# rbesenczi/newMSM

Measured on AMD Instinct MI355X. Metric: label-cost evals/sec, higher is better.
Workload: dtype f64; 1 GPU; pairwise sulc (D=1) unary label-cost table, ico6 data grid / ico4 control grid, 19 labels, 48678 evals = 3187573 point samples per step (BASELINE config 2); kind=univariate, simmeasure=correlation, replicas=1

## Files before the change

### newmsm_amd/csrc/cost.cpp

```cpp
#include <algorithm>
#include <chrono>
#include <cmath>
#include <cstdio>
#include <cstdlib>
#include <cstring>

#include "cost_internal.hpp"
#include "host_parallel.hpp"

using namespace msm;

namespace msm {
int ensure_vertex_major(msm_cost *c) {
    if (c->vm_valid) return MSM_OK;
    msm_ctx *ctx = c->ctx;
    const int Ns = c->source->V, D = c->D, R = c->cfw_rows;
    std::vector<double> vm((size_t)Ns * D);
    for (int d = 0; d < D; ++d)
        for (int v = 0; v < Ns; ++v) vm[(size_t)v * D + d] = c->sfeat[(size_t)d * Ns + v];
    MSM_HIP(c->d_sfeat_vm.ensure(vm.size()));
    {
        const int st = upload_staged(ctx, c->d_sfeat_vm.p, vm.data(), sizeof(double) * vm.size());
        if (st) return st;
    }
// ... 144 lines not shown
    MSM_HIP(c->d_absw.ensure(N));
    st = upload_staged(ctx, c->d_maxw.p, mw.data(), sizeof(double) * (size_t)Ns);
    if (st) return st;
    st = apply_weights_dev(ctx, w, c->d_maxw.p, 1, c->d_absw.p);
    if (st) return st;
    c->absw.resize(N);
    MSM_TRY(stage_d2h(ctx, c->absw.data(), c->d_absw.p, sizeof(double) * (size_t)N));
    MSM_TRY(ctx_sync(ctx));
    return MSM_OK;
}

int ensure_unary_table(msm_cost *c) {
    if (c->table_valid) return MSM_OK;
    int st = need(c, c->have_source, "get_source_data()");
    if (st) return st;
    st = need(c, c->L > 0, "labels");
    if (st) return st;
    st = need(c, c->target->d_feat.p != nullptr && c->target->D == c->D, "target features matching the source features");
    if (st) return st;
    msm_ctx *ctx = c->ctx;
    const int N = c->cpgrid->V;
    MSM_HIP(c->d_U.ensure((size_t)c->L * N));
    if (is_ho(c)) {
        MSM_HIP(hipMemsetAsync(c->d_U.p, 0, sizeof(double) * (size_t)c->L * N, ctx->stream));
        c->table_valid = true;
        return MSM_OK;
    }
    st = ensure_rays(c->target);
    if (st) return st;
    UnaryLaunch u;
    u.tree = dev_tree(c->target);
    u.tfeat = c->target->d_feat.p;
    u.D = c->D;
    u.N = N;
    u.L = c->L;
    u.cp = c->cpgrid->d_xyz.p;
    st = ensure_label_rotations(c);
    if (st) return st;
    u.rnl = c->d_rnl.p;
    u.labels = c->d_labels.p;
    u.src = c->source->d_xyz.p;
    u.Nsrc = c->source->V;
    u.sfeat = c->d_sfeat.p;
    u.cfw = c->cfw.empty() ? nullptr : c->d_cfw.p;
    u.cfw_rows = c->cfw_rows;
    u.pptr = c->d_pptr.p;
    u.pidx = c->d_pidx.p;
    u.order = c->d_order.p;
    u.absw = c->d_absw.p;
    u.pmax = c->pmax;
    u.simmeasure = c->p.simmeasure;
    u.percentile = c->p.percentile;
    u.U = c->d_U.p;
    const size_t nsamp = (size_t)c->L * c->pidx.size();
    MSM_HIP(c->d_tval.ensure(nsamp));
    MSM_HIP(c->d_fix_list.ensure(nsamp));
    MSM_HIP(c->d_fix_pt.ensure(3 * nsamp));
    if (!c->d_fix_count.p) MSM_HIP(c->d_fix_count.zero(unary_fix_counter_words(), ctx->stream));
    if (!c->fix_off_valid) {
        std::vector<uint32_t> off;
        unary_fix_offsets(N, c->L, c->pmax, c->pptr.data(), c->order.data(), off);
        MSM_TRY(c->d_fix_off.upload(off.data(), off.size(), ctx));
        MSM_TRY(ctx_sync(ctx));
        c->fix_off_valid = true;
    }
    MSM_HIP(c->d_queues.ensure(N));
    u.ntri = c->target->T;
    u.tval = c->d_tval.p;
    u.fix_list = c->d_fix_list.p;
    u.fix_pt = c->d_fix_pt.p;
    u.fix_cnt = c->d_fix_count.p;
    u.fix_off = c->d_fix_off.p;
    u.redo_list = c->d_queues.p;
    if (c->timing) {
        u.ev_start = c->ev0[c->ev_next];
        u.ev_stop = c->ev1[c->ev_next];
        c->ev_next = (c->ev_next + 1) % (int)c->ev0.size();
        c->ev_count = std::min(c->ev_count + 1, (int)c->ev0.size());
    }
    switch (c->p.kind) {
        case MSM_COST_UNIVARIATE: st = launch_unary_univariate(ctx, u); break;
        case MSM_COST_MULTIVARIATE:
        case MSM_COST_PATCHWISE: {
            {
                st = ensure_vertex_major(c);
                if (st) return st;
                u.sfeat_vm = c->d_sfeat_vm.p;
                u.cfw_vm = c->cfw.empty() ? nullptr : c->d_cfw_vm.p;
            }
            MSM_HIP(c->d_stri.ensure(nsamp));
            MSM_HIP(c->d_sw3.ensure(3 * nsamp));
            UnaryWeightsScratch w{c->d_stri.p, c->d_sw3.p};
            st = launch_unary_multivariate(ctx, u, w, c->p.kind == MSM_COST_PATCHWISE);
            break;
        }
        default: return fail(MSM_ERR_INVALID, "unknown cost kind %d", c->p.kind);
    }
    if (st) return st;
    c->counters[0] += (int64_t)nsamp;
    c->counters[1] += (int64_t)c->L * N;
    c->table_valid = true;
    return MSM_OK;
}

}

extern "C" {

msm_cost *msm_cost_create(msm_ctx *ctx, const msm_cost_params *params) {
    if (!ctx || !params) {
        fail(MSM_ERR_INVALID, "msm_cost_create: null argument");
        return nullptr;
    }
    if (params->kind < MSM_COST_UNIVARIATE || params->kind > MSM_COST_HO_MULTIVARIATE) {
        fail(MSM_ERR_INVALID, "msm_cost_create: unknown cost kind %d", params->kind);
        return nullptr;
    }
    if (params->simmeasure != 1 && params->simmeasure != 2 && params->simmeasure != 4 && params->simmeasure != 5) {
        fail(MSM_ERR_INVALID, "Unknown similarity metric");
        return nullptr;
    }
    if ((params->simmeasure == 4 || params->simmeasure == 5) && !(params->percentile > 0.0 + kEps && params->percentile < 1.0 - kEps)) {
        fail(MSM_ERR_INVALID, "Percentile must be between 0 and 1.");
        return nullptr;
    }
    msm_cost *c = new msm_cost();
    c->ctx = ctx;
    c->p = *params;
    (void)hipSetDevice(ctx->device);
    if (c->d_counters.zero(4, ctx->stream) != hipSuccess) {
        fail(MSM_ERR_HIP, "msm_cost_create: allocation failed");
        delete c;
        return nullptr;
    }
// ... 221 lines not shown
    if (st) return st;
    if (ngroups) *ngroups = c->ngroups;
    if (ptr) std::copy(c->pptr.begin(), c->pptr.end(), ptr);
    if (idx) {
        if ((int64_t)c->pidx.size() > cap) return fail(MSM_ERR_CAPACITY, "patch index buffer too small");
        std::copy(c->pidx.begin(), c->pidx.end(), idx);
    }
    return MSM_OK;
}

int msm_cost_absolute_weights(msm_cost *c, double *absw) {
    if (!c || !absw) return fail(MSM_ERR_INVALID, "msm_cost_absolute_weights: null argument");
    int st = need(c, c->have_source, "get_source_data()");
    if (st) return st;
    std::copy(c->absw.begin(), c->absw.end(), absw);
    return MSM_OK;
}

int msm_cost_unary_table_async(msm_cost *c) {
    if (!c) return fail(MSM_ERR_INVALID, "null cost");
    MSM_TRY(drop_ctx_pending(c->ctx));
    c->table_valid = false;
    c->rotations_valid = false;
    c->h_U.clear();
    return ensure_unary_table(c);
}

int msm_cost_unary_table_fetch(msm_cost *c, double *U) {
    if (!c || !U) return fail(MSM_ERR_INVALID, "msm_cost_unary_table_fetch: null argument");
    MSM_TRY(drop_ctx_pending(c->ctx));
    int st = need(c, c->table_valid, "msm_cost_unary_table_async()");
    if (st) return st;
    msm_ctx *ctx = c->ctx;
    const size_t n = (size_t)c->L * c->cpgrid->V;
    void *mapped = ctx_mapped(ctx, U, sizeof(double) * n);
    if (mapped && reinterpret_cast<uintptr_t>(mapped) % 16 == 0) {
        st = ctx_flag(ctx);
        if (st) return st;
        st = launch_copy_to_mapped(ctx, c->d_U.p, static_cast<double *>(mapped), n, ctx->d_flag_map);
        if (st) return st;
        MSM_TRY(ctx_sync(ctx));
        volatile int *flags = ctx->h_flag;
        if (flags[0] != 0) {
            flags[0] = 0;
            return check_status(ctx, "computeUnaryCosts");
        }
        return MSM_OK;
    }
    MSM_TRY(c->d_U.download(U, n, ctx));
    return check_status(ctx, "computeUnaryCosts");
}

int msm_cost_unary_table(msm_cost *c, double *U) {
    int st = msm_cost_unary_table_async(c);
    if (st) return st;
    return msm_cost_unary_table_fetch(c, U);
}

int msm_cost_unary_batch(msm_cost *c, const int32_t *nodes, const int32_t *labels, int32_t n, double *out) {
    if (!c || !nodes || !labels || !out || n < 0) return fail(MSM_ERR_INVALID, "msm_cost_unary_batch: bad arguments");
    MSM_TRY(drop_ctx_pending(c->ctx));
    if (!c->table_valid || c->h_U.size() != (size_t)c->L * c->cpgrid->V) {
        int st = ensure_unary_table(c);
        if (st) return st;
        c->h_U.resize((size_t)c->L * c->cpgrid->V);
        st = msm_cost_unary_table_fetch(c, c->h_U.data());
        if (st) return st;
    }
    const int N = c->cpgrid->V;
    for (int i = 0; i < n; ++i) {
        if (nodes[i] < 0 || nodes[i] >= N || labels[i] < 0 || labels[i] >= c->L) return fail(MSM_ERR_INVALID, "unary query %d out of range", i);
        out[i] = c->h_U[(size_t)labels[i] * N + nodes[i]];
    }
    return MSM_OK;
}

int msm_cost_enable_timing(msm_cost *c, int enable) {
    if (!c) return fail(MSM_ERR_INVALID, "null cost");
    if (enable && c->ev0.empty()) {
        c->ev0.resize(64);
        c->ev1.resize(64);
        for (size_t i = 0; i < c->ev0.size(); ++i) {
            MSM_HIP(hipEventCreate(&c->ev0[i]));
            MSM_HIP(hipEventCreate(&c->ev1[i]));
        }
    }
    c->timing = enable != 0;
    c->ev_next = 0;
    c->ev_count = 0;
    return MSM_OK;
}

int msm_cost_kernel_times(msm_cost *c, double *ms, int32_t cap, int32_t *n) {
    if (!c || !ms || !n) return fail(MSM_ERR_INVALID, "msm_cost_kernel_times: null argument");
    MSM_TRY(drop_ctx_pending(c->ctx));
    MSM_TRY(ctx_sync(c->ctx));
    const int total = (int)c->ev0.size(), cnt = std::min(c->ev_count, (int)cap);
    for (int k = 0; k < cnt; ++k) {
        const int slot = ((c->ev_next - cnt + k) % total + total) % total;
        float f = 0.f;
        MSM_HIP(hipEventElapsedTime(&f, c->ev0[slot], c->ev1[slot]));
        ms[k] = f;
    }
    *n = cnt;
    return MSM_OK;
}

int msm_cost_counters(msm_cost *c, int64_t counters[4]) {
    if (!c || !counters) return fail(MSM_ERR_INVALID, "msm_cost_counters: null argument");
// ... 10 lines not shown
```

### newmsm_amd/csrc/cost_internal.hpp

```cpp
#pragma once

#include <vector>

#include "devbuf.hpp"
#include "kernels.hpp"

using msm::DevBuf;

struct msm_cost {
    msm_ctx *ctx = nullptr;
    msm_cost_params p{};
    msm_mesh *target = nullptr, *source = nullptr, *cpgrid = nullptr;
    std::vector<double> orig_xyz;
    std::vector<double> ocp_xyz;
    int D = 0;
    std::vector<double> sfeat;
    DevBuf<double> d_sfeat;
    DevBuf<double> d_sfeat_vm, d_cfw_vm;
    bool vm_valid = false;
    std::vector<double> cfw;
    int cfw_rows = 0;
    DevBuf<double> d_cfw;
    std::vector<double> maxsep;
    double mvdmax = 0;
    DevBuf<double> d_maxsep;
    int L = 0;
    std::vector<double> labels, rot;
    DevBuf<double> d_labels, d_rot;
    DevBuf<double> d_rnl, d_moved;
    std::vector<int32_t> triplets, pairs;
    DevBuf<int32_t> d_triplets, d_pairs;
    DevBuf<double> d_orig, d_ocp;
    DevBuf<int32_t> d_cp_tri, d_cp_tid_ptr, d_cp_tid;
    bool cp_conn_valid = false;
    DevBuf<int32_t> d_labeling;
    DevBuf<double> d_clique_out;
    DevBuf<double> d_ho_vals, d_ho_big;
    DevBuf<unsigned> d_ho_pending, d_ho_count;
    DevBuf<int32_t> d_slot_tri;
    DevBuf<int4> d_blk;
    DevBuf<double> d_slot_w, d_slot_sf, d_slot_cw, d_slot_wda, d_tri_frame, d_tri_stat;
    int64_t move_tails = 0;
    struct PendingMove {
        bool valid = false;
        int kind = 0;
        int label = 0;
        double *E = nullptr;
        uint64_t epoch = 0;
        std::vector<int32_t> labeling;
        msm::CliqueArgs a;
        msm::MoveArgs m;
        msm::MoveLabels lab;
    } pending;
    int64_t prefetch_hits = 0, prefetch_drops = 0;
    DevBuf<unsigned> d_defer_list, d_defer_cnt;
    int move_nblk = 0, move_cap = 0, move_parity = 0;
    bool move_valid = false;
    bool have_source = false;
    int ngroups = 0, pmax = 0;
    std::vector<int32_t> pptr, pidx;
    DevBuf<int32_t> d_pptr, d_pidx;
    std::vector<int32_t> order;
    DevBuf<int32_t> d_order;
    DevBuf<uint32_t> d_fix_off;
    bool fix_off_valid = false;
    std::vector<double> absw;
    DevBuf<int32_t> d_pidx_asc;
    DevBuf<uint32_t> d_code;
    DevBuf<double4> d_chunkb;
    bool pidx_asc_on_device = false;
    int patch_cap_hint = 0;
    DevBuf<double> d_absw, d_maxw;
    DevBuf<double> d_U;
    bool table_valid = false;
    bool rotations_valid = false;
    std::vector<double> h_U;
    DevBuf<unsigned long long> d_counters;
    int64_t counters[4] = {0, 0, 0, 0};
    DevBuf<uint32_t> d_slots;
    DevBuf<double> d_tval;
    DevBuf<int> d_stri;
    DevBuf<double> d_sw3;
    DevBuf<unsigned long long> d_fix_list;
    DevBuf<double> d_fix_pt;
    DevBuf<unsigned int> d_fix_count;
    msm_mesh *asphere = nullptr;
    int aVs = 0, aTs = 0;
    DevBuf<double> d_atarget, d_asrc, d_aw_val;
    DevBuf<int32_t> d_asrc_tri, d_aw_ptr, d_aw_cp, d_af_ptr, d_af_idx;
    bool have_anat = false;
    bool timing = false;
    std::vector<hipEvent_t> ev0, ev1;
    int ev_next = 0, ev_count = 0;
    DevBuf<int> d_queues;
    DevBuf<int> d_counts;
};


namespace msm {
int query_host(msm_mesh *target, const double *q, int N, int *tri_id, int *vid, double *w, int mode, const char *what, const double *q_on_device = nullptr);
const Adjacency &mesh_adjacency(msm_mesh *m);
int ensure_label_rotations(msm_cost *c);
int drop_pending_move(msm_cost *c);
int ensure_vertex_major(msm_cost *c);
inline bool cost_is_ho(const msm_cost *c) { return c->p.kind == MSM_COST_HO_UNIVARIATE || c->p.kind == MSM_COST_HO_MULTIVARIATE; }
}
```

### newmsm_amd/csrc/internal.hpp

```cpp
#pragma once

#include <hip/hip_runtime.h>

#include <cstdarg>
#include <cstdint>
#include <cstdio>
#include <functional>
#include <memory>
#include <mutex>
#include <string>
#include <vector>

#include "../../include/msmhip.h"
#include "devbuf.hpp"
#include "geom.hpp"

namespace msm {

void set_error(const char *fmt, ...);
int fail(int code, const char *fmt, ...);
void pool_trim();
size_t pool_idle_bytes();

#define MSM_HIP(call)                                                                                 \
// ... 30 lines not shown
    bool simple = false;
    int G = 0;
    std::vector<int4> cell;
    std::vector<float4> edge;
    std::vector<int4> more;
    std::vector<int4> excl;
    double r2lo = 0, r2hi = 0;
};

struct FlatOctree {
    std::vector<int4> node;
    std::vector<double4> nodebox;
    int nmask_blocks = 0;
    std::vector<int32_t> parent;
    std::vector<int32_t> leaf_tri;
    std::vector<int32_t> grid;
    int grid_depth = 0;
    RayTable rays;
    int64_t stats[5] = {0, 0, 0, 0, 0};
    int dev_nnodes = 0, dev_entries = 0;
    int nnodes() const { return node.empty() ? dev_nnodes : (int)node.size(); }
    int nentries() const { return node.empty() ? dev_entries : (int)leaf_tri.size(); }
};
void build_octree(const double *xyz , const int32_t *tri , int V, int T, FlatOctree &out);
void build_ray_table(const double *xyz, const int32_t *tri, int V, int T, FlatOctree &tree);

struct DevTree {
    const int4 *node;
    const int32_t *parent;
    const int32_t *leaf_tri;
    const float4 *cone;
    const TriRec *rec;
    const int32_t *grid;
    int grid_depth;
    int simple;
    const unsigned long long *mask;
    int nnodes;
    int ray_G;
    const int4 *ray_cell;
    const float4 *ray_tri;
    const int4 *ray_more, *ray_excl;
    double ray_r2lo, ray_r2hi;
};

}

namespace msm {
struct Stager;
}

struct msm_ctx {
    int device = 0;
    int num_cus = 256;
    hipStream_t stream = nullptr;
    bool own_stream = false;
    int *d_status = nullptr;
    int *h_status = nullptr;
    msm::DevBuf<char> q_buf[5];
    msm::Stager *stager = nullptr;
    hipEvent_t wait_ev = nullptr;
    struct msm_cost *pending_cost = nullptr;
    uint64_t epoch = 0;
    void *io_pin = nullptr;
    void *io_dev = nullptr;
    size_t io_cap = 0;
    int *h_flag = nullptr;
    int *d_flag_map = nullptr;
    std::shared_ptr<void> resample_scratch;
    hipEvent_t q_ev0 = nullptr, q_ev1 = nullptr;
    bool q_timing = false, q_timed = false;
    msm::DevBuf<double> oct_box;
    msm::DevBuf<int> oct_ints, oct_counters;
    int *oct_hcounters = nullptr;
    struct HostBlock {
        char *host;
        char *dev;
        size_t bytes;
        bool registered = false;
    };
    std::vector<HostBlock> host_blocks;
};

namespace msm {
struct RayJob;
}

struct msm_mesh {
    msm_ctx *ctx = nullptr;
    int V = 0, T = 0, D = 0;
    std::vector<double> xyz;
    std::vector<int32_t> tri;
    std::vector<double> feat;
    bool tree_valid = false;
    bool gpu_tree_always = false;
    bool host_xyz_stale = false;
    std::shared_ptr<void> oct_job;
    msm::FlatOctree tree;
    bool masks_valid = false;
    bool rays_valid = false;
    bool rayrec_valid = false;
    msm::Adjacency adj;
    bool adj_valid = false;
    msm::DevBuf<double> d_xyz;
    msm::DevBuf<int32_t> d_tri;
    msm::DevBuf<float4> d_tcone;
    msm::DevBuf<double> d_feat;
// ... 84 lines not shown
```

### newmsm_amd/csrc/kernels.hpp

```cpp
#pragma once

#include "internal.hpp"

namespace msm {

int launch_build_masks(msm_ctx *ctx, const DevTree &T, const double4 *d_nodebox, unsigned long long *d_mask);
int launch_build_recs(msm_ctx *ctx, const double *d_xyz, int V, const int32_t *d_tri, int T, TriRec *d_rec, float4 *d_tcone, const int32_t *d_leaf_tri,
                      int nentries, float4 *d_cone);
int launch_build_recs_forest(msm_ctx *ctx, const double *d_xyz, size_t comp_stride, size_t tree_stride, const int32_t *d_tri, int T, int B, TriRec *d_rec, float4 *d_tcone,
                             size_t s_rec, const int32_t *d_leaf_tri, float4 *d_cone, size_t s_leaf, const int *d_entries, size_t entries_stride);
int launch_build_raytri(msm_ctx *ctx, const TriRec *d_rec, const float4 *d_edge, int T, const double *d_feat1, int D, float4 *d_out);
struct AdaptiveDevArgs {
    int nOld, nNew;
    const int *fvid, *rvid;
    const double *fw, *rw;
    const double *oldA, *newA;
    int *roff, *rfill, *rkey;
    double *rwt;
    int *coff, *cfill, *ckey;
    double *cval, *correction;
    int *scan_tmp;
    int *long_flag;
    int *tkey;
    double *tval;
// ... 9 lines not shown
int launch_vertex_areas(msm_ctx *ctx, const double *d_xyz, int V, const int32_t *d_tri, int T, const int32_t *d_tid_ptr, const int32_t *d_tid, double *d_ta,
                        double *d_area);
int launch_adaptive_surgery(msm_ctx *ctx, const AdaptiveDevArgs &a);
int launch_apply_rows(msm_ctx *ctx, int nNew, int nOld, int D, const int *row_ptr, const int *col, const double *val, const double *d_data, double *d_out);
int launch_copy_to_mapped(msm_ctx *ctx, const double *d_src, double *mapped_dst, size_t n, int *flags_mapped);
int launch_query(msm_ctx *ctx, const DevTree &T, const double *d_q, int N, int *d_tri, int *d_vid, double *d_w, int mode);
int launch_query_rays(msm_ctx *ctx, const DevTree &T, const double *d_q, int N, int *d_tri, int *d_vid, double *d_w, int mode, int *d_open);
int launch_closest_vertex(msm_ctx *ctx, const DevTree &T, const double *d_q, int N, int *d_out);
int launch_warp(msm_ctx *ctx, const DevTree &T, const double *d_q, int N, const double *d_to, int V, bool to_sphere, double *d_out);
int query_lanes(long long N);
inline size_t smooth_bounds_offset(int N) { return ((size_t)3 * N + 3) / 4 * 4; }
inline size_t smooth_scratch_doubles(int N) { return smooth_bounds_offset(N) + 4 * (((size_t)N + 63) / 64) + 4; }
int launch_smooth(msm_ctx *ctx, const double *d_xyz, int N, double *d_unit, const int *d_cv, const double *d_data, int Vorig, int D, double sigma,
                  double cosang, const double *d_excl, double *d_out, double *d_excl_out);
int launch_fold_detect(msm_ctx *ctx, const double *d_xyz, int V, const int32_t *d_tri, int T, const int32_t *d_tid_ptr, const int32_t *d_tid, int32_t *d_fold);
int launch_sort_patches(msm_ctx *ctx, const double *d_xyz, int n, const int32_t *d_pptr, int ngroups, const int32_t *d_pidx, uint32_t *d_code,
                        int32_t *d_sorted);
struct RangeGrid {
    const int *start = nullptr, *ids = nullptr, *bad = nullptr;
    int G = 0;
    double origin = 0.0, inv_h = 0.0;
};
int launch_range_grid_build(msm_ctx *ctx, const double *d_src, int Nsrc, int G, double origin, double inv_h, int *d_start, int *d_cursor, int *d_ids, int *d_bad, int *d_tmp);
int launch_range(msm_ctx *ctx, const double *d_cp, int Ncp, const double *d_src, int Nsrc, const double *d_maxsep, double range, int cap,
                 uint32_t *d_slots, int *d_counts, double4 *d_chunk_bounds, int *d_nflag, int cluster = 1, const RangeGrid *grid = nullptr);
int launch_patch_compact(msm_ctx *ctx, const uint32_t *d_slots, int cap, const int32_t *d_pptr, int M, int32_t *d_pidx, size_t pidx_cap = (size_t)-1);
int launch_scan_exclusive(msm_ctx *ctx, int *d_data, int n, int *d_tmp);

int launch_label_rotations(msm_ctx *ctx, const double *d_cp, int N, const double *d_rot, const double *d_labels, int L, double *d_rnl,
                           double *d_moved);

struct UnaryLaunch {
    DevTree tree;
    const double *tfeat;
    int D;
    int N, L;
    const double *cp;
    const double *rnl;
    const double *labels;
    const double *src;
    int Nsrc;
    const double *sfeat;
    const double *cfw;
    int cfw_rows;
    const double *sfeat_vm = nullptr;
    const double *cfw_vm = nullptr;
    const int *pptr, *pidx;
    const int *order;
    const double *absw;
    int pmax;
    int simmeasure;
    double percentile;
    double *U;
    int ntri;
    double *tval;
    unsigned long long *fix_list;
    double *fix_pt;
    unsigned int *fix_cnt;
    const unsigned int *fix_off;
    int *redo_list;
    hipEvent_t ev_start = nullptr, ev_stop = nullptr;
};
int unary_nsplit(int L, int pmax);
int unary_fix_segments();
size_t unary_fix_counter_words();
void unary_fix_offsets(int N, int L, int pmax, const int32_t *pptr, const int32_t *order, std::vector<uint32_t> &off);
int launch_unary_univariate(msm_ctx *ctx, const UnaryLaunch &u);
struct UnaryWeightsScratch {
    int *stri;
    double *sw3;
};
int launch_unary_multivariate(msm_ctx *ctx, const UnaryLaunch &u, const UnaryWeightsScratch &w, bool patchwise);

struct CliqueArgs {
    int kind, simmeasure;
    int N, L, T, P;
    const int *triplets;
    const int *pairs;
    const double *cp;
    const double *ocp;
    const double *orig;
    int Norig;
    const double *moved;
    const double *rnl;
    const int *cp_tri;
    int Tc;
    const int *cp_tid_ptr, *cp_tid;
    double lambda, mu, kappa, k_exp, rexp, mvdmax, percentile;
    DevTree tree;
    const double *tfeat;
    int D;
    const double *src;
    int Nsrc;
    const double *sfeat;
    const double *cfw;
    int cfw_rows;
    const double *sfeat_vm, *cfw_vm;
    const int *bin_ptr, *bin_idx;
    int bin_cap;
    double *ho_big;
    double *ho_vals;
    unsigned *ho_pending;
    unsigned *ho_count;
    const double *absw;
    int rmode;
    DevTree atree;
    const double *atarget;
    int Va;
    const double *asrc;
    int Vs;
    const int *asrc_tri;
    int Ts;
    const int *aw_ptr, *aw_cp;
    const double *aw_val;
    const int *af_ptr, *af_idx;
    int *status;
};
constexpr int kPairSmallPatch = 80;
constexpr int kHoBinMax = 16384;
constexpr int kHoBigBlocks = 512;
// ... 102 lines not shown
```

### newmsm_amd/csrc/unary_kernels.hip

```cpp
#include <algorithm>
#include <cstdlib>

#include "kernels.hpp"
#include "search_device.hpp"
#include "similarity_device.hpp"

#ifndef MSM_VARIANT
#define MSM_VARIANT 0
#endif

namespace msm {

namespace {

constexpr int kFixSegs = 64;
constexpr int kCntStride = 32;
constexpr int kChunk = 768;
constexpr int kQueueCap = 3072;
constexpr int kDeferred = 1 << 20;
constexpr unsigned kInvalidPair = 0xffffffffu;
constexpr int kTriBits = 22;

__device__ __forceinline__ void raise_status(int *status, int code) { atomicMin(status, code); }

__device__ __forceinline__ double wave_sum(double v) {
#pragma unroll
    for (int off = 32; off > 0; off >>= 1) v += __shfl_xor(v, off, 64);
    return v;
}

struct SamplesArgs {
    DevTree tree;
    const double *tfeat;
    int tD;
    int N, L;
    const double *rnl;
    const double *src;
    int Nsrc;
    const int *pptr, *pidx;
    const int *order;
    int pmax;
    int nsplit;
    double *tval;
    int *stri;
    double *sw3;
    unsigned long long *fix_list;
    double *fix_pt;
    unsigned int *fix_cnt;
    const unsigned int *fix_off;
    const double *sfeat;
    const double *cfw;
    const double *absw;
    int simmeasure;
    double percentile;
    double *U;
    int *redo_list;
    unsigned int *redo_count;
    int *status;
// ... 422 lines not shown
            else emit_sample(a, g, p, t);
        }
    }
}

struct ReduceArgs {
    int N, L, Nsrc;
    const double *sfeat;
    const double *cfw;
    int cfw_rows;
    const int *pptr, *pidx;
    const double *absw;
    const double *tval;
    int pmax;
    int simmeasure;
    double percentile;
    double *U;
    const int *redo_list;
    const unsigned int *redo_count;
};

__global__ __launch_bounds__(256) void k_unary_reduce_univariate(ReduceArgs a) {
    extern __shared__ __align__(16) double lds[];
    double *sA = lds, *sW = sA + a.pmax;
    const int tid = threadIdx.x, lane = tid & 63, wave = tid >> 6;
    const unsigned n = a.redo_count ? *a.redo_count : (unsigned)a.N;
    for (unsigned k = blockIdx.x; k < n; k += gridDim.x) {
        const int node = a.redo_list ? a.redo_list[k] : (int)k;
        const int beg = a.pptr[node], P = a.pptr[node + 1] - beg;
        __syncthreads();
        for (int i = tid; i < P; i += 256) {
            const int s = a.pidx[beg + i];
            sA[i] = a.sfeat[s];
            sW[i] = (a.cfw && a.cfw_rows >= 1) ? a.cfw[s] : 1.0;
        }
        __syncthreads();
        const double absw = a.absw[node];
        for (int l = wave; l < a.L; l += 4) {
            const double cost = patch_similarity(sA, sW, a.tval + (size_t)a.L * beg + (size_t)l * P, P, lane, a.simmeasure, a.percentile);
            if (lane == 0) a.U[(size_t)l * a.N + node] = absw * cost;
        }
    }
}

constexpr int kRedLanes = 8;
constexpr int kRedKeep = 12;

__device__ __forceinline__ double group_sum(double v) {
#pragma unroll
    for (int off = kRedLanes / 2; off > 0; off >>= 1) v += __shfl_xor(v, off, kRedLanes);
    return v;
}

__global__ __launch_bounds__(256) void k_unary_reduce_flat(ReduceArgs a, unsigned int *clear, int clear_words) {
    extern __shared__ __align__(16) double lds[];
    double *sA = lds, *sW = sA + a.pmax;
    __shared__ double s_stat[3];
    const int tid = threadIdx.x, sub = tid & (kRedLanes - 1), grp = tid / kRedLanes;
    if (blockIdx.x == 0 && clear)
        for (int k = tid; k < clear_words; k += 256) clear[k] = 0u;
    const int node = a.redo_list ? a.redo_list[blockIdx.x] : (int)blockIdx.x;
    const int beg = a.pptr[node], P = a.pptr[node + 1] - beg;
    const bool has_w = a.cfw && a.cfw_rows >= 1;
    const bool in_regs = true;
    double breg[kRedKeep];
#pragma unroll
    for (int k = 0; k < kRedKeep; ++k) breg[k] = 0.0;
    if (grp < a.L) {
        const double *B = a.tval + (size_t)a.L * beg + (size_t)grp * P;
#pragma unroll
        for (int k = 0; k < kRedKeep; ++k) breg[k] = (sub + kRedLanes * k < P) ? B[sub + kRedLanes * k] : 0.0;
    }
    for (int i = tid; i < P; i += 256) {
        const int s = a.pidx[beg + i];
        sA[i] = a.sfeat[s];
        sW[i] = has_w ? a.cfw[s] : 1.0;
    }
    __syncthreads();
    if (a.simmeasure == 2) {
        if (tid < 64) {
            double sw = 0, ma = 0;
            for (int i = tid; i < P; i += 64) {
                sw += sW[i];
                ma += sW[i] * sA[i];
            }
            sw = wave_sum(sw);
            ma = wave_sum(ma);
            if (sw > 0.0) ma /= sw;
            double va = 0;
            for (int i = tid; i < P; i += 64) {
                const double da = sA[i] - ma;
                va += sW[i] * da * da;
            }
            va = wave_sum(va);
            if (tid == 0) s_stat[0] = sw, s_stat[1] = ma, s_stat[2] = va;
        }
        __syncthreads();
    }
    const double absw = a.absw[node];
    for (int l = grp; l < a.L; l += 256 / kRedLanes) {
        const double *B = a.tval + (size_t)a.L * beg + (size_t)l * P;
        if (!(in_regs && l == grp)) {
#pragma unroll
            for (int k = 0; k < kRedKeep; ++k) breg[k] = (sub + kRedLanes * k < P) ? B[sub + kRedLanes * k] : 0.0;
        }
        double cost;
        if (a.simmeasure == 2) {
            const double sw = s_stat[0], ma = s_stat[1];
            double mb = 0;
#pragma unroll
            for (int k = 0; k < kRedKeep; ++k) {
                const int i = sub + kRedLanes * k;
                if (i < P) mb += sW[i] * breg[k];
            }
            for (int i = sub + kRedLanes * kRedKeep; i < P; i += kRedLanes) mb += sW[i] * B[i];
            mb = group_sum(mb);
            if (sw > 0.0) mb /= sw;
            double pr = 0, vb = 0;
#pragma unroll
            for (int k = 0; k < kRedKeep; ++k) {
                const int i = sub + kRedLanes * k;
                if (i < P) {
                    const double da = sA[i] - ma, db = breg[k] - mb;
                    pr += sW[i] * da * db;
                    vb += sW[i] * db * db;
                }
            }
            for (int i = sub + kRedLanes * kRedKeep; i < P; i += kRedLanes) {
                const double da = sA[i] - ma, db = B[i] - mb;
                pr += sW[i] * da * db;
                vb += sW[i] * db * db;
            }
            pr = group_sum(pr);
            vb = group_sum(vb);
            double va = s_stat[2];
            if (sw > 0.0) {
                pr /= sw;
                va /= sw;
                vb /= sw;
            }
            const double r = (va == 0.0 || vb == 0.0) ? 0.0 : pr / (sqrt(va) * sqrt(vb));
            cost = 1 - (1 + r) * 0.5;
        } else {
            double pr = 0;
#pragma unroll
            for (int k = 0; k < kRedKeep; ++k) {
                const int i = sub + kRedLanes * k;
                if (i < P) {
                    const double df = sA[i] - breg[k];
                    pr += sW[i] * df * df;
                }
            }
            for (int i = sub + kRedLanes * kRedKeep; i < P; i += kRedLanes) {
                const double df = sA[i] - B[i];
                pr += sW[i] * df * df;
            }
            pr = group_sum(pr);
            cost = sqrt(pr) / P;
        }
        if (sub == 0) a.U[(size_t)l * a.N + node] = absw * cost;
    }
}

struct ReduceMvArgs {
    int N, L, Nsrc, D;
    const double *tfeat;
    const TriRec *rec;
    const double *sfeat;
    const double *cfw;
    int cfw_rows;
    const int *pptr, *pidx;
    const double *absw;
    const int *stri;
    const double *sw3;
    int simmeasure;
    double percentile;
    int patchwise;
    int pmax;
    double *U;
};

__global__ __launch_bounds__(256) void k_unary_reduce_features(ReduceMvArgs a) {
    const int node = blockIdx.x;
    const int beg = a.pptr[node], P = a.pptr[node + 1] - beg;
    const int tid = threadIdx.x, lane = tid & 63, wave = tid >> 6;
    const double absw = a.absw[node];
    const double nan = __longlong_as_double(0x7ff8000000000000ll);
    const int nwaves = blockDim.x >> 6;
    for (int l = wave; l < a.L; l += nwaves) {
        const size_t g0 = (size_t)a.L * beg + (size_t)l * P;
        double cost;
        if (!a.patchwise) {
            double acc = 0.0;
            bool bad = false;
            for (int i = lane; i < P; i += 64) {
                const int t = a.stri[g0 + i];
                if (t < 0) {
                    bad = true;
                    continue;
                }
                const TriRec &r = a.rec[t];
                const double *f0 = a.tfeat + (size_t)r.id[0] * a.D, *f1 = a.tfeat + (size_t)r.id[1] * a.D, *f2 = a.tfeat + (size_t)r.id[2] * a.D;
                acc += feature_vector_similarity(a.simmeasure, a.percentile, a.sfeat, a.cfw, a.cfw_rows, a.Nsrc, a.pidx[beg + i], a.D, f0, f1, f2,
                                                 a.sw3[3 * (g0 + i)], a.sw3[3 * (g0 + i) + 1], a.sw3[3 * (g0 + i) + 2]);
            }
            acc = wave_sum(acc);
            cost = P > 0 ? acc / P : acc;
            if (__ballot(bad)) cost = nan;
        } else {
            double total = 0.0;
            bool bad = false;
            for (int d = 0; d < a.D; ++d) {
                const double *A = a.sfeat + (size_t)d * a.Nsrc;
// ... 275 lines not shown

static bool uses_ray_table(const DevTree &t) { return t.simple && t.ray_G > 0 && t.ray_cell && t.ray_tri; }

static int launch_samples(msm_ctx *ctx, const UnaryLaunch &u, const UnaryWeightsScratch *w, SamplesArgs &a, bool fused_reduction = false) {
    if (u.tree.nnodes <= 0 || !u.tree.mask) return fail(MSM_ERR_STATE, "target search structure missing");
    a.tree = u.tree;
    a.tfeat = u.tfeat;
    a.tD = u.D > 0 ? u.D : 1;
    a.N = u.N;
    a.L = u.L;
    a.rnl = u.rnl;
    a.src = u.src;
    a.Nsrc = u.Nsrc;
    a.pptr = u.pptr;
    a.pidx = u.pidx;
    a.order = u.order;
    a.pmax = u.pmax;
    a.tval = w ? nullptr : u.tval;
    a.stri = w ? w->stri : nullptr;
    a.sw3 = w ? w->sw3 : nullptr;
    a.fix_list = u.fix_list;
    a.fix_pt = u.fix_pt;
    a.fix_cnt = u.fix_cnt;
    a.fix_off = u.fix_off;
    a.sfeat = u.sfeat;
    a.cfw = (u.cfw && u.cfw_rows >= 1) ? u.cfw : nullptr;
    a.absw = u.absw;
    a.simmeasure = u.simmeasure;
    a.percentile = u.percentile;
    a.U = (w || !fused_reduction) ? nullptr : u.U;
    a.redo_list = u.redo_list;
    a.redo_count = u.fix_cnt;
    a.status = ctx->d_status;
    if (u.ntri >= (1 << kTriBits)) return fail(MSM_ERR_CAPACITY, "target mesh has %d triangles; the sample queue packs ids in %d bits", u.ntri, kTriBits);
    a.nsplit = unary_nsplit(u.L, u.pmax);
    const size_t lds = samples_lds(u.pmax, u.L, a.nsplit);
    if (!uses_ray_table(u.tree) && lds > 64 * 1024) {
        if (lds > 160 * 1024) return fail(MSM_ERR_CAPACITY, "a patch of %d points does not fit in LDS", u.pmax);
        MSM_HIP(hipFuncSetAttribute(reinterpret_cast<const void *>(k_unary_samples), hipFuncAttributeMaxDynamicSharedMemorySize, (int)lds));
    }
    const int blocks = a.nsplit * 8 * ((u.N + 7) / 8);
    if (u.ev_start) MSM_HIP(hipEventRecord(u.ev_start, ctx->stream));
    if (uses_ray_table(u.tree)) {
        a.U = nullptr;
        const int lper = (u.L + a.nsplit - 1) / a.nsplit;
        const size_t rays_lds = sizeof(double) * (3 * (size_t)u.pmax + 9 * (size_t)u.L) + sizeof(int) * ((size_t)lper * u.pmax + 4) + 16;
        if (rays_lds > 64 * 1024) MSM_HIP(hipFuncSetAttribute(reinterpret_cast<const void *>(k_unary_rays), hipFuncAttributeMaxDynamicSharedMemorySize, (int)rays_lds));
        hipLaunchKernelGGL(k_unary_rays, dim3(blocks), dim3(256), rays_lds, ctx->stream, a);
    } else {
        hipLaunchKernelGGL(k_unary_samples, dim3(blocks), dim3(256), lds, ctx->stream, a);
    }
    MSM_HIP(hipGetLastError());
    if (u.ev_stop) MSM_HIP(hipEventRecord(u.ev_stop, ctx->stream));
    hipLaunchKernelGGL(k_unary_fixup, dim3(4096), dim3(256), 0, ctx->stream, a);
    MSM_HIP(hipGetLastError());
    return MSM_OK;
}

int launch_unary_univariate(msm_ctx *ctx, const UnaryLaunch &u) {
    SamplesArgs a;
    const bool dice = u.simmeasure == 4 || u.simmeasure == 5;
    int st = launch_samples(ctx, u, nullptr, a, dice);
    if (st) return st;
    ReduceArgs r;
    r.N = u.N;
    r.L = u.L;
    r.Nsrc = u.Nsrc;
    r.sfeat = u.sfeat;
    r.cfw = u.cfw;
    r.cfw_rows = u.cfw_rows;
    r.pptr = u.pptr;
    r.pidx = u.pidx;
    r.absw = u.absw;
    r.tval = u.tval;
    r.pmax = u.pmax;
    r.simmeasure = u.simmeasure;
    r.percentile = u.percentile;
    r.U = u.U;
    r.redo_list = u.redo_list;
    r.redo_count = u.fix_cnt;
    if (uses_ray_table(u.tree) && dice) {
        r.redo_list = nullptr;
        r.redo_count = nullptr;
        hipLaunchKernelGGL(k_unary_reduce_univariate, dim3(std::min(u.N, 2048)), dim3(256), sizeof(double) * 2 * (size_t)u.pmax, ctx->stream, r);
        MSM_HIP(hipMemsetAsync(u.fix_cnt, 0, unary_fix_counter_words() * sizeof(unsigned), ctx->stream));
    } else if (!dice) {
        r.redo_list = u.order;
        hipLaunchKernelGGL(k_unary_reduce_flat, dim3(u.N), dim3(256), sizeof(double) * 2 * (size_t)u.pmax, ctx->stream, r, u.fix_cnt,
                           (int)unary_fix_counter_words());
    } else {
        hipLaunchKernelGGL(k_unary_reduce_univariate, dim3(64), dim3(256), sizeof(double) * 2 * (size_t)u.pmax, ctx->stream, r);
        MSM_HIP(hipMemsetAsync(u.fix_cnt, 0, unary_fix_counter_words() * sizeof(unsigned), ctx->stream));
    }
    MSM_HIP(hipGetLastError());
    return MSM_OK;
}

int launch_unary_multivariate(msm_ctx *ctx, const UnaryLaunch &u, const UnaryWeightsScratch &w, bool patchwise) {
    SamplesArgs a;
    int st = launch_samples(ctx, u, &w, a);
    if (st) return st;
    ReduceMvArgs r;
    r.N = u.N;
    r.L = u.L;
    r.Nsrc = u.Nsrc;
    r.D = u.D;
    r.tfeat = u.tfeat;
    r.rec = u.tree.rec;
    r.sfeat = u.sfeat;
    r.cfw = u.cfw;
    r.cfw_rows = u.cfw_rows;
    r.pptr = u.pptr;
    r.pidx = u.pidx;
    r.absw = u.absw;
    r.stri = w.stri;
    r.sw3 = w.sw3;
    r.simmeasure = u.simmeasure;
    r.patchwise = patchwise ? 1 : 0;
    r.pmax = u.pmax;
    r.percentile = u.percentile;
    r.U = u.U;
    const bool dice = u.simmeasure == 4 || u.simmeasure == 5;
    if (!dice && u.D >= 12 && u.D <= kMvLanes * kMvKeep && u.sfeat_vm) {
        ReduceMv8Args m;
        m.N = u.N, m.L = u.L, m.Nsrc = u.Nsrc, m.D = u.D;
        m.tfeat = u.tfeat;
        m.rec = u.tree.rec;
        m.sfeat_vm = u.sfeat_vm;
        m.cfw_vm = u.cfw_vm;
        m.cfw_rows = u.cfw_rows;
        m.pptr = u.pptr, m.pidx = u.pidx, m.order = u.order;
        m.absw = u.absw;
        m.stri = w.stri, m.sw3 = w.sw3;
        m.simmeasure = u.simmeasure;
        m.U = u.U;
        if (!patchwise) hipLaunchKernelGGL(k_unary_reduce_mv8, dim3(u.N), dim3(256), 0, ctx->stream, m);
        else if (u.D <= 32) hipLaunchKernelGGL(k_unary_reduce_pw8<4>, dim3(u.N), dim3(256), 0, ctx->stream, m);
        else hipLaunchKernelGGL(k_unary_reduce_pw8<8>, dim3(u.N), dim3(256), 0, ctx->stream, m);
// ... 18 lines not shown
```

Baseline: 367.2 million evals/s.

## Tile univariate reduce across nodes and write table directly to mapped host memory

Adds a k_unary_finish kernel that reduces several control nodes per block, staging per-label costs in LDS and prefetching the next row's samples into registers. It also clears the fixup counters and reports status, replacing the separate reduce launch and memset. When the caller's output buffer is host-mapped, the kernel writes results straight into it, skipping the separate copy-to-mapped launch or download. The fixup kernel grid is now sized to resident occupancy instead of a fixed 4096 blocks. The cost is that the whole table is written over system memory from the kernel, and the new kernel uses more LDS per block.

New measurement: 355.6 million evals/s. -3.2%, worse.

```diff
diff --git a/newmsm_amd/csrc/cost.cpp b/newmsm_amd/csrc/cost.cpp
--- a/newmsm_amd/csrc/cost.cpp
+++ b/newmsm_amd/csrc/cost.cpp
@@ -220,6 +220,9 @@
     u.simmeasure = c->p.simmeasure;
     u.percentile = c->p.percentile;
     u.U = c->d_U.p;
+    u.U_mapped = c->deliver_to;
+    u.flag_mapped = ctx->d_flag_map;
+    c->delivered = false;
     const size_t nsamp = (size_t)c->L * c->pidx.size();
     MSM_HIP(c->d_tval.ensure(nsamp));
     MSM_HIP(c->d_fix_list.ensure(nsamp));
@@ -247,7 +250,7 @@
         c->ev_count = std::min(c->ev_count + 1, (int)c->ev0.size());
     }
     switch (c->p.kind) {
-        case MSM_COST_UNIVARIATE: st = launch_unary_univariate(ctx, u); break;
+        case MSM_COST_UNIVARIATE: st = launch_unary_univariate(ctx, u, &c->delivered); break;
         case MSM_COST_MULTIVARIATE:
         case MSM_COST_PATCHWISE: {
             {
@@ -575,9 +578,29 @@
 }
 
 int msm_cost_unary_table(msm_cost *c, double *U) {
+    if (!c || !U) return fail(MSM_ERR_INVALID, "msm_cost_unary_table: null argument");
+    msm_ctx *ctx = c->ctx;
+    c->deliver_to = nullptr;
+    c->delivered = false;
+    if (c->cpgrid && c->L > 0) {
+        void *mapped = ctx_mapped(ctx, U, sizeof(double) * (size_t)c->L * c->cpgrid->V);
+        if (mapped && reinterpret_cast<uintptr_t>(mapped) % 16 == 0) {
+            int st = ctx_flag(ctx);
+            if (st) return st;
+            c->deliver_to = static_cast<double *>(mapped);
+        }
+    }
     int st = msm_cost_unary_table_async(c);
-    if (st) return st;
-    return msm_cost_unary_table_fetch(c, U);
+    c->deliver_to = nullptr;
+    if (st) return st;
+    if (!c->delivered) return msm_cost_unary_table_fetch(c, U);
+    MSM_TRY(ctx_sync(ctx));
+    volatile int *flags = ctx->h_flag;
+    if (flags[0] != 0) {
+        flags[0] = 0;
+        return check_status(ctx, "computeUnaryCosts");
+    }
+    return MSM_OK;
 }
 
 int msm_cost_unary_batch(msm_cost *c, const int32_t *nodes, const int32_t *labels, int32_t n, double *out) {
diff --git a/newmsm_amd/csrc/cost_internal.hpp b/newmsm_amd/csrc/cost_internal.hpp
--- a/newmsm_amd/csrc/cost_internal.hpp
+++ b/newmsm_amd/csrc/cost_internal.hpp
@@ -74,6 +74,8 @@
     DevBuf<double> d_U;
     bool table_valid = false;
     bool rotations_valid = false;
+    double *deliver_to = nullptr;
+    bool delivered = false;
     std::vector<double> h_U;
     DevBuf<unsigned long long> d_counters;
     int64_t counters[4] = {0, 0, 0, 0};
diff --git a/newmsm_amd/csrc/internal.hpp b/newmsm_amd/csrc/internal.hpp
--- a/newmsm_amd/csrc/internal.hpp
+++ b/newmsm_amd/csrc/internal.hpp
@@ -106,6 +106,7 @@
 struct msm_ctx {
     int device = 0;
     int num_cus = 256;
+    int unary_fixup_blocks = 0;
     hipStream_t stream = nullptr;
     bool own_stream = false;
     int *d_status = nullptr;
diff --git a/newmsm_amd/csrc/kernels.hpp b/newmsm_amd/csrc/kernels.hpp
--- a/newmsm_amd/csrc/kernels.hpp
+++ b/newmsm_amd/csrc/kernels.hpp
@@ -85,6 +85,8 @@
     int simmeasure;
     double percentile;
     double *U;
+    double *U_mapped = nullptr;
+    int *flag_mapped = nullptr;
     int ntri;
     double *tval;
     unsigned long long *fix_list;
@@ -98,7 +100,7 @@
 int unary_fix_segments();
 size_t unary_fix_counter_words();
 void unary_fix_offsets(int N, int L, int pmax, const int32_t *pptr, const int32_t *order, std::vector<uint32_t> &off);
-int launch_unary_univariate(msm_ctx *ctx, const UnaryLaunch &u);
+int launch_unary_univariate(msm_ctx *ctx, const UnaryLaunch &u, bool *delivered = nullptr);
 struct UnaryWeightsScratch {
     int *stri;
     double *sw3;
diff --git a/newmsm_amd/csrc/unary_kernels.hip b/newmsm_amd/csrc/unary_kernels.hip
--- a/newmsm_amd/csrc/unary_kernels.hip
+++ b/newmsm_amd/csrc/unary_kernels.hip
@@ -4,6 +4,7 @@
 #include "kernels.hpp"
 #include "search_device.hpp"
 #include "similarity_device.hpp"
+#include "unary_shape.hpp"
 
 #ifndef MSM_VARIANT
 #define MSM_VARIANT 0
@@ -532,6 +533,88 @@
     return v;
 }
 
+__device__ __forceinline__ void flat_patch_stats(const double *sA, const double *sW, int P, int lane, double *stat) {
+    double sw = 0, ma = 0;
+    for (int i = lane; i < P; i += 64) {
+        sw += sW[i];
+        ma += sW[i] * sA[i];
+    }
+    sw = wave_sum(sw);
+    ma = wave_sum(ma);
+    if (sw > 0.0) ma /= sw;
+    double va = 0;
+    for (int i = lane; i < P; i += 64) {
+        const double da = sA[i] - ma;
+        va += sW[i] * da * da;
+    }
+    va = wave_sum(va);
+    if (lane == 0) stat[0] = sw, stat[1] = ma, stat[2] = va;
+}
+
+__device__ __forceinline__ void flat_row_load(double (&breg)[kRedKeep], const double *B, int P, int sub) {
+#pragma unroll
+    for (int k = 0; k < kRedKeep; ++k) breg[k] = (sub + kRedLanes * k < P) ? B[sub + kRedLanes * k] : 0.0;
+}
+
+__device__ __forceinline__ double flat_row_cost(int simmeasure, const double *sA, const double *sW, const double (&breg)[kRedKeep], const double *B, int P,
+                                                int sub, const double *stat) {
+    double cost;
+    if (simmeasure == 2) {
+        const double sw = stat[0], ma = stat[1];
+        double mb = 0;
+#pragma unroll
+        for (int k = 0; k < kRedKeep; ++k) {
+            const int i = sub + kRedLanes * k;
+            if (i < P) mb += sW[i] * breg[k];
+        }
+        for (int i = sub + kRedLanes * kRedKeep; i < P; i += kRedLanes) mb += sW[i] * B[i];
+        mb = group_sum(mb);
+        if (sw > 0.0) mb /= sw;
+        double pr = 0, vb = 0;
+#pragma unroll
+        for (int k = 0; k < kRedKeep; ++k) {
+            const int i = sub + kRedLanes * k;
+            if (i < P) {
+                const double da = sA[i] - ma, db = breg[k] - mb;
+                pr += sW[i] * da * db;
+                vb += sW[i] * db * db;
+            }
+        }
+        for (int i = sub + kRedLanes * kRedKeep; i < P; i += kRedLanes) {
+            const double da = sA[i] - ma, db = B[i] - mb;
+            pr += sW[i] * da * db;
+            vb += sW[i] * db * db;
+        }
+        pr = group_sum(pr);
+        vb = group_sum(vb);
+        double va = stat[2];
+        if (sw > 0.0) {
+            pr /= sw;
+            va /= sw;
+            vb /= sw;
+        }
+        const double r = (va == 0.0 || vb == 0.0) ? 0.0 : pr / (sqrt(va) * sqrt(vb));
+        cost = 1 - (1 + r) * 0.5;
+    } else {
+        double pr = 0;
+#pragma unroll
+        for (int k = 0; k < kRedKeep; ++k) {
+            const int i = sub + kRedLanes * k;
+            if (i < P) {
+                const double df = sA[i] - breg[k];
+                pr += sW[i] * df * df;
+            }
+        }
+        for (int i = sub + kRedLanes * kRedKeep; i < P; i += kRedLanes) {
+            const double df = sA[i] - B[i];
+            pr += sW[i] * df * df;
+        }
+        pr = group_sum(pr);
+        cost = sqrt(pr) / P;
+    }
+    return cost;
+}
+
 __global__ __launch_bounds__(256) void k_unary_reduce_flat(ReduceArgs a, unsigned int *clear, int clear_words) {
     extern __shared__ __align__(16) double lds[];
     double *sA = lds, *sW = sA + a.pmax;
@@ -547,9 +630,7 @@
 #pragma unroll
     for (int k = 0; k < kRedKeep; ++k) breg[k] = 0.0;
     if (grp < a.L) {
-        const double *B = a.tval + (size_t)a.L * beg + (size_t)grp * P;
-#pragma unroll
-        for (int k = 0; k < kRedKeep; ++k) breg[k] = (sub + kRedLanes * k < P) ? B[sub + kRedLanes * k] : 0.0;
+        flat_row_load(breg, a.tval + (size_t)a.L * beg + (size_t)grp * P, P, sub);
     }
     for (int i = tid; i < P; i += 256) {
         const int s = a.pidx[beg + i];
@@ -558,87 +639,108 @@
     }
     __syncthreads();
     if (a.simmeasure == 2) {
-        if (tid < 64) {
-            double sw = 0, ma = 0;
-            for (int i = tid; i < P; i += 64) {
-                sw += sW[i];
-                ma += sW[i] * sA[i];
-            }
-            sw = wave_sum(sw);
-            ma = wave_sum(ma);
-            if (sw > 0.0) ma /= sw;
-            double va = 0;
-            for (int i = tid; i < P; i += 64) {
-                const double da = sA[i] - ma;
-                va += sW[i] * da * da;
-            }
-            va = wave_sum(va);
-            if (tid == 0) s_stat[0] = sw, s_stat[1] = ma, s_stat[2] = va;
-        }
+        if (tid < 64) flat_patch_stats(sA, sW, P, tid, s_stat);
         __syncthreads();
     }
     const double absw = a.absw[node];
     for (int l = grp; l < a.L; l += 256 / kRedLanes) {
         const double *B = a.tval + (size_t)a.L * beg + (size_t)l * P;
-        if (!(in_regs && l == grp)) {
-#pragma unroll
-            for (int k = 0; k < kRedKeep; ++k) breg[k] = (sub + kRedLanes * k < P) ? B[sub + kRedLanes * k] : 0.0;
-        }
-        double cost;
-        if (a.simmeasure == 2) {
-            const double sw = s_stat[0], ma = s_stat[1];
-            double mb = 0;
-#pragma unroll
-            for (int k = 0; k < kRedKeep; ++k) {
-                const int i = sub + kRedLanes * k;
-                if (i < P) mb += sW[i] * breg[k];
-            }
-            for (int i = sub + kRedLanes * kRedKeep; i < P; i += kRedLanes) mb += sW[i] * B[i];
-            mb = group_sum(mb);
-            if (sw > 0.0) mb /= sw;
-            double pr = 0, vb = 0;
-#pragma unroll
-            for (int k = 0; k < kRedKeep; ++k) {
-                const int i = sub + kRedLanes * k;
-                if (i < P) {
-                    const double da = sA[i] - ma, db = breg[k] - mb;
-                    pr += sW[i] * da * db;
-                    vb += sW[i] * db * db;
-                }
-            }
-            for (int i = sub + kRedLanes * kRedKeep; i < P; i += kRedLanes) {
-                const double da = sA[i] - ma, db = B[i] - mb;
-                pr += sW[i] * da * db;
-                vb += sW[i] * db * db;
-            }
-            pr = group_sum(pr);
-            vb = group_sum(vb);
-            double va = s_stat[2];
-            if (sw > 0.0) {
-                pr /= sw;
-                va /= sw;
-                vb /= sw;
-            }
-            const double r = (va == 0.0 || vb == 0.0) ? 0.0 : pr / (sqrt(va) * sqrt(vb));
-            cost = 1 - (1 + r) * 0.5;
+        if (!(in_regs && l == grp)) flat_row_load(breg, B, P, sub);
+        const double cost = flat_row_cost(a.simmeasure, sA, sW, breg, B, P, sub, s_stat);
+        if (sub == 0) a.U[(size_t)l * a.N + node] = absw * cost;
+    }
+}
+
+struct FinishOut {
+    double *mapped;
+    const int *status;
+    int *flags;
+    unsigned int *clear;
+    int clear_words;
+};
+
+#ifndef MSM_FINISH_TILE
+#define MSM_FINISH_TILE 8
+#endif
+constexpr int kFinishTile = MSM_FINISH_TILE;
+
+template <int TILE>
+__global__ __launch_bounds__(64 * TILE, 4) void k_unary_finish(ReduceArgs a, FinishOut o) {
+    extern __shared__ __align__(16) double lds[];
+    constexpr int kGroups = 8 * TILE, kThreads = 64 * TILE;
+    double *sU = lds, *sStat = sU + (size_t)a.L * TILE, *sA = sStat + 4 * TILE, *sW = sA + (size_t)TILE * a.pmax;
+    const int tid = threadIdx.x, sub = tid & (kRedLanes - 1), grp = tid / kRedLanes, lane = tid & 63, wave = tid >> 6;
+    if (blockIdx.x == 0) {
+        for (int k = tid; k < o.clear_words; k += kThreads) o.clear[k] = 0u;
+        if (o.mapped && tid == 0) {
+            const int st = *o.status;
+            if (st != 0) __hip_atomic_store(o.flags, st, __ATOMIC_RELAXED, __HIP_MEMORY_SCOPE_SYSTEM);
+        }
+    }
+    const int node0 = blockIdx.x * TILE, nt = min(TILE, a.N - node0), rows = nt * a.L;
+    const int beg0 = a.pptr[node0];
+    const bool has_w = a.cfw && a.cfw_rows >= 1;
+    int w = 0, l = 0, off = 0, P = 0;
+    const double *B = a.tval;
+    auto locate = [&](int r) {
+        w = r / a.L;
+        l = r - w * a.L;
+        const int beg = a.pptr[node0 + w];
+        P = a.pptr[node0 + w + 1] - beg;
+        off = beg - beg0;
+        B = a.tval + (size_t)a.L * beg + (size_t)l * P;
+    };
+    double breg[kRedKeep], bnext[kRedKeep];
+#pragma unroll
+    for (int k = 0; k < kRedKeep; ++k) breg[k] = bnext[k] = 0.0;
+    if (grp < rows) {
+        locate(grp);
+        flat_row_load(breg, B, P, sub);
+    }
+    const int total = a.pptr[node0 + nt] - beg0;
+    for (int i = tid; i < total; i += kThreads) {
+        const int s = a.pidx[beg0 + i];
+        sA[i] = a.sfeat[s];
+        sW[i] = has_w ? a.cfw[s] : 1.0;
+    }
+    __syncthreads();
+    if (a.simmeasure == 2) {
+        for (int k = wave; k < nt; k += TILE) {
+            const int beg = a.pptr[node0 + k];
+            flat_patch_stats(sA + (beg - beg0), sW + (beg - beg0), a.pptr[node0 + k + 1] - beg, lane, sStat + 4 * k);
+        }
+        __syncthreads();
+    }
+    for (int r = grp; r < rows; r += kGroups) {
+        const int w_now = w, l_now = l, off_now = off, P_now = P;
+        const double *B_now = B;
+        if (r + kGroups < rows) {
+            locate(r + kGroups);
+            flat_row_load(bnext, B, P, sub);
+        }
+        const double cost = flat_row_cost(a.simmeasure, sA + off_now, sW + off_now, breg, B_now, P_now, sub, sStat + 4 * w_now);
+        if (sub == 0) sU[l_now * TILE + w_now] = a.absw[node0 + w_now] * cost;
+#pragma unroll
+        for (int k = 0; k < kRedKeep; ++k) breg[k] = bnext[k];
+    }
+    __syncthreads();
+    for (int t = tid; t < a.L * (TILE / 2); t += kThreads) {
+        const int ls = t / (TILE / 2), h = t - ls * (TILE / 2);
+        const size_t at = (size_t)ls * a.N + node0 + 2 * h;
+        const double2 v = *reinterpret_cast<const double2 *>(sU + ls * TILE + 2 * h);
+        if (unary_finish_wide_store(ls, a.N, node0, nt, TILE)) {
+            *reinterpret_cast<double2 *>(a.U + at) = v;
+            if (o.mapped) *reinterpret_cast<double2 *>(o.mapped + at) = v;
         } else {
-            double pr = 0;
-#pragma unroll
-            for (int k = 0; k < kRedKeep; ++k) {
-                const int i = sub + kRedLanes * k;
-                if (i < P) {
-                    const double df = sA[i] - breg[k];
-                    pr += sW[i] * df * df;
-                }
-            }
-            for (int i = sub + kRedLanes * kRedKeep; i < P; i += kRedLanes) {
-                const double df = sA[i] - B[i];
-                pr += sW[i] * df * df;
-            }
-            pr = group_sum(pr);
-            cost = sqrt(pr) / P;
-        }
-        if (sub == 0) a.U[(size_t)l * a.N + node] = absw * cost;
+            if (2 * h < nt) {
+                a.U[at] = v.x;
+                if (o.mapped) o.mapped[at] = v.x;
+            }
+            if (2 * h + 1 < nt) {
+                a.U[at + 1] = v.y;
+                if (o.mapped) o.mapped[at + 1] = v.y;
+            }
+        }
     }
 }
 
@@ -1020,12 +1122,18 @@
     }
     MSM_HIP(hipGetLastError());
     if (u.ev_stop) MSM_HIP(hipEventRecord(u.ev_stop, ctx->stream));
-    hipLaunchKernelGGL(k_unary_fixup, dim3(4096), dim3(256), 0, ctx->stream, a);
+    if (ctx->unary_fixup_blocks <= 0) {
+        int per_cu = 0;
+        MSM_HIP(hipOccupancyMaxActiveBlocksPerMultiprocessor(&per_cu, reinterpret_cast<const void *>(k_unary_fixup), 256, 0));
+        ctx->unary_fixup_blocks = unary_resident_blocks(ctx->num_cus, per_cu);
+    }
+    hipLaunchKernelGGL(k_unary_fixup, dim3(ctx->unary_fixup_blocks), dim3(256), 0, ctx->stream, a);
     MSM_HIP(hipGetLastError());
     return MSM_OK;
 }
 
-int launch_unary_univariate(msm_ctx *ctx, const UnaryLaunch &u) {
+int launch_unary_univariate(msm_ctx *ctx, const UnaryLaunch &u, bool *delivered) {
+    if (delivered) *delivered = false;
     SamplesArgs a;
     const bool dice = u.simmeasure == 4 || u.simmeasure == 5;
     int st = launch_samples(ctx, u, nullptr, a, dice);
@@ -1052,6 +1160,17 @@
         r.redo_count = nullptr;
         hipLaunchKernelGGL(k_unary_reduce_univariate, dim3(std::min(u.N, 2048)), dim3(256), sizeof(double) * 2 * (size_t)u.pmax, ctx->stream, r);
         MSM_HIP(hipMemsetAsync(u.fix_cnt, 0, unary_fix_counter_words() * sizeof(unsigned), ctx->stream));
+    } else if (!dice && sizeof(double) * unary_finish_lds_doubles(u.L, u.pmax, kFinishTile) <= 64 * 1024) {
+        r.redo_list = nullptr;
+        FinishOut o;
+        o.mapped = u.U_mapped;
+        o.status = ctx->d_status;
+        o.flags = u.flag_mapped;
+        o.clear = u.fix_cnt;
+        o.clear_words = (int)unary_fix_counter_words();
+        hipLaunchKernelGGL(k_unary_finish<kFinishTile>, dim3(unary_finish_tiles(u.N, kFinishTile)), dim3(64 * kFinishTile),
+                           sizeof(double) * unary_finish_lds_doubles(u.L, u.pmax, kFinishTile), ctx->stream, r, o);
+        if (delivered) *delivered = u.U_mapped != nullptr;
     } else if (!dice) {
         r.redo_list = u.order;
         hipLaunchKernelGGL(k_unary_reduce_flat, dim3(u.N), dim3(256), sizeof(double) * 2 * (size_t)u.pmax, ctx->stream, r, u.fix_cnt,
diff --git a/newmsm_amd/csrc/unary_shape.hpp b/newmsm_amd/csrc/unary_shape.hpp
--- /dev/null
+++ b/newmsm_amd/csrc/unary_shape.hpp
@@ -0,0 +1,27 @@
+#pragma once
+
+#include <cstddef>
+
+#if defined(__HIPCC__)
+#define MSM_SHAPE_FN __host__ __device__ inline
+#else
+#define MSM_SHAPE_FN inline
+#endif
+
+namespace msm {
+
+MSM_SHAPE_FN int unary_resident_blocks(int cus, int blocks_per_cu) {
+    const int c = cus > 0 ? cus : 1, b = blocks_per_cu > 0 ? blocks_per_cu : 1;
+    const long long n = (long long)c * b;
+    return n > 65536 ? 65536 : (int)n;
+}
+
+MSM_SHAPE_FN int unary_finish_tiles(int N, int tile) { return N > 0 ? (N + tile - 1) / tile : 0; }
+
+MSM_SHAPE_FN size_t unary_finish_lds_doubles(int L, int pmax, int tile) { return (size_t)tile * ((size_t)L + 4 + 2 * (size_t)pmax); }
+
+MSM_SHAPE_FN bool unary_finish_wide_store(int l, int N, int node0, int nt, int tile) {
+    return nt == tile && (tile & 1) == 0 && ((((size_t)l * (size_t)N + (size_t)node0) & 1) == 0);
+}
+
+}
```
